# suous/RecNeXt

Hardware: AMD Instinct MI355X
Metric: images/sec RecNeXt-M3 224x224 bf16 (higher is better)
Workload: dtype bf16

## Files before the change

### recnext_amd/csrc/rcx_api.hip

```cpp
#include "../../include/recnext_amd.h"
#include "rcx_opts.h"
#include "rcx_launch.h"

#include <cstdarg>
#include <initializer_list>
#include <cstdio>
#include <cstdlib>

namespace {

thread_local char g_err[512] = "";

int fail(int code, const char* fmt, ...)
{
    va_list ap;
    va_start(ap, fmt);
    vsnprintf(g_err, sizeof(g_err), fmt, ap);
    va_end(ap);
    return code;
}

int hip_fail(hipError_t e, const char* what, const char* prefix = "")
{
    snprintf(g_err, sizeof(g_err), "%s%s: %s", prefix, what, hipGetErrorString(e));
// ... 548 lines not shown
}

size_t rcx_recconv2d_train_saved_bytes(int N, int C, int H, int W, int level, int k)
{
    if (!bwd_extents_ok(N, C, H, W, level, k)) return 0;
    return make_train_ladder(N, C, H, W, level, k).saved_total;
}

size_t rcx_recconv2d_bwd_workspace_bytes(int N, int C, int H, int W, int level, int k)
{
    if (!bwd_extents_ok(N, C, H, W, level, k)) return 0;
    return make_train_ladder(N, C, H, W, level, k).bwd_total;
}

int rcx_recconv2d_fwd_train(const void* x, void* y, const float* wpack, const float* bpack, void* saved, size_t saved_bytes,
                            int N, int C, int H, int W, int level, int k, int mode, int dtype, void* stream)
{
    if (int rc = check_common(x, y, N, C, H, W, k, dtype)) return rc;
    if (!wpack) return fail(RCX_ERR_BAD_ARG, "null weight pack");
    if (level < 0 || level > RCX_MAX_LEVEL) return fail(RCX_ERR_BAD_ARG, "level %d outside [0,%d]", level, RCX_MAX_LEVEL);
    if (mode != RCX_MODE_BILINEAR && mode != RCX_MODE_NEAREST) return fail(RCX_ERR_BAD_ARG, "unknown mode %d", mode);
    const TrainLadder L = make_train_ladder(N, C, H, W, level, k);
    if (L.saved_total > 0 && (!saved || saved_bytes < L.saved_total))
        return fail(RCX_ERR_WORKSPACE, "saved-activation buffer too small: need %zu bytes, got %zu", L.saved_total, saved_bytes);
    hipStream_t s = (hipStream_t)stream;
    const int md = mode == RCX_MODE_NEAREST ? 1 : 0;
    const TrainFwdSchedule sch = train_fwd_schedule(N, C, H, W, level, k, mode, dtype);
    if (sch == TRAIN_STEPS) return recconv2d_steps(x, y, wpack, bpack, (char*)saved, L.f_off, L.c_off, L.h, L.w, N, C, level, k, mode, dtype, s, "train fwd: ");
    const hipError_t e = sch == TRAIN_TILED ? rcx::cpt_recconv(x, y, wpack, bpack, N, C, H, level, md, dtype, s, (float*)saved, L.f_off, L.c_off)
                       : sch == TRAIN_CPL14 ? rcx::cpl14_recconv(x, y, wpack, bpack, N, C, md, dtype, s, (float*)saved, L.f_off, L.c_off)
                                            : rcx::cpl7b_recconv(x, y, wpack, bpack, N, C, md, dtype, s, (float*)saved, L.f_off, L.c_off);
    static const char* const what[] = {"train fwd: fused tiled block", "train fwd: fused 14x14 block", "train fwd: fused 7x7 block"};
    return e == hipSuccess ? 0 : hip_fail(e, what[sch]);
}

int rcx_recconv2d_bwd_gy_dtype(int N, int C, int H, int W, int level, int k, int dtype)
{
    if (!bwd_extents_ok(N, C, H, W, level, k) || !known_dtype(dtype)) return RCX_DTYPE_F32;
    if (dtype != RCX_DTYPE_BF16 || C % 4) return RCX_DTYPE_F32;
    return bwd_schedule(make_train_ladder(N, C, H, W, level, k), N, C, level, k, dtype, true).kind != BWD_STEPS ? dtype : RCX_DTYPE_F32;
}

const char* rcx_recconv2d_bwd_plan(int N, int C, int H, int W, int level, int k, int dtype)
{
    static thread_local char desc[64];
    return bwd_plan(desc, N, C, H, W, level, k, dtype, true, "k_recconv_bwd_");
}

int rcx_recconv2d_bwd(const void* x, const void* gy, int gy_dtype, const float* wpack, const float* wpack_flipped, const void* saved,
                      void* gx, float* gwpack, float* gbpack, void* const* gw_out, void* const* gb_out, int grad_dtype,
                      void* workspace, size_t workspace_bytes,
                      int N, int C, int H, int W, int level, int k, int mode, int dtype, void* stream)
{
    if (int rc = check_common(x, gx, N, C, H, W, k, dtype)) return rc;
    if (!gy || !wpack || !wpack_flipped || (!gwpack && !gw_out)) return fail(RCX_ERR_BAD_ARG, "null gradient / weight pointer");
    if (gw_out && !known_dtype(grad_dtype)) return fail(RCX_ERR_BAD_ARG, "unknown gradient dtype %d", grad_dtype);
    if (int rc = check_bwd_args(gy_dtype, C, level, mode)) return rc;
    const TrainLadder L = make_train_ladder(N, C, H, W, level, k);
    if (level >= 1 && !saved) return fail(RCX_ERR_BAD_ARG, "null saved-activation buffer");
    if (!workspace || workspace_bytes < L.bwd_total)
        return fail(RCX_ERR_WORKSPACE, "backward workspace too small: need %zu bytes, got %zu", L.bwd_total, workspace_bytes);
    const BwdSchedule sch = bwd_schedule(L, N, C, level, k, dtype, true);
    if (gy_dtype != RCX_DTYPE_F32 && !(sch.kind != BWD_STEPS && gy_dtype == dtype && dtype == RCX_DTYPE_BF16))
        return fail(RCX_ERR_UNSUPPORTED, "gy of dtype %d: this problem takes float32 (rcx_recconv2d_bwd_gy_dtype)", gy_dtype);
    if (gw_out)
        for (int i = 0; i < level + 2; ++i)
            if (!gw_out[i]) return fail(RCX_ERR_BAD_ARG, "null gw_out[%d]", i);
    hipStream_t s = (hipStream_t)stream;
    BwdRun B{L, true, "bwd: "};
    B.x = x; B.gy = gy; B.wpack = wpack; B.wflip = wpack_flipped; B.saved = (const char*)saved; B.ws = (char*)workspace; B.gx = gx;
    B.gy_dt = gy_dtype; B.N = N; B.C = C; B.level = level; B.k = k; B.mode = mode; B.dtype = dtype; B.s = s;
    rcx::WgradJobs& J = B.J;
    J.njobs = level + 2; J.kk = k * k; J.C = C; J.param_layout = gw_out ? 1 : 0; J.param_dt = grad_dtype;
    for (int i = 0; i < level + 2; ++i) {
        J.gw[i] = gw_out ? (float*)gw_out[i] : gwpack + (size_t)i * k * k * C;
        J.gb[i] = gw_out ? (gb_out ? (float*)gb_out[i] : nullptr) : (gbpack ? gbpack + (size_t)i * C : nullptr);
    }
    if (sch.kind == BWD_ONE) RCX_TRY(one_launch(B, gy, gy_dtype, gx, 0, H, level, dtype), "fused block", B.prefix);
    else if (int rc = sch.kind == BWD_TILED ? bwd_tiled(B, sch.m) : bwd_steps(B, sch.m)) return rc;
    float* const gw0 = J.gw[0], * const gb0 = J.gb[0];
    if (level == 0) { J.njobs = 1; J.gw[0] = J.gw[1]; J.gb[0] = J.gb[1]; J.nslots[0] = J.nslots[1]; J.part[0][0] = J.part[1][0]; J.rows[0][0] = J.rows[1][0]; }
    RCX_TRY(rcx::bwd_wgrad_reduce_jobs(J, s), "weight-gradient reduction", B.prefix);
    if (level >= 1) return 0;
    const size_t esz = gw_out && grad_dtype != RCX_DTYPE_F32 ? 2 : 4;
    hipError_t e = hipMemsetAsync(gw0, 0, esz * k * k * C, s);
    if (e == hipSuccess && gb0) e = hipMemsetAsync(gb0, 0, esz * C, s);
    return e == hipSuccess ? 0 : hip_fail(e, "bwd: zero down grad");
}

size_t rcx_recconv2d_bwd_input_workspace_bytes(int N, int C, int H, int W, int level, int k)
{
    if (!bwd_extents_ok(N, C, H, W, level, k)) return 0;
    const TrainLadder L = make_train_ladder(N, C, H, W, level, k);
    return bwd_input_workspace(L, bwd_schedule(L, N, C, level, k, RCX_DTYPE_F32, false).kind);
}

int rcx_recconv2d_bwd_input_gy_dtype(int N, int C, int H, int W, int level, int k, int dtype)
{
    if (!bwd_extents_ok(N, C, H, W, level, k) || !known_dtype(dtype) || dtype == RCX_DTYPE_F32 || C % 4) return RCX_DTYPE_F32;
    return bwd_schedule(make_train_ladder(N, C, H, W, level, k), N, C, level, k, dtype, false).kind != BWD_STEPS ? dtype : RCX_DTYPE_F32;
}

const char* rcx_recconv2d_bwd_input_plan(int N, int C, int H, int W, int level, int k, int dtype)
{
    static thread_local char desc[64];
    return bwd_plan(desc, N, C, H, W, level, k, dtype, false, "k_recconv_adj_");
}

int rcx_recconv2d_bwd_input(const void* gy, int gy_dtype, const float* wpack, const float* wpack_flipped, void* gx,
                            void* workspace, size_t workspace_bytes,
                            int N, int C, int H, int W, int level, int k, int mode, int dtype, void* stream)
{
    if (int rc = check_common(gy, gx, N, C, H, W, k, dtype)) return rc;
    if (!wpack || !wpack_flipped) return fail(RCX_ERR_BAD_ARG, "null weight pack");
    if (gy == gx) return fail(RCX_ERR_BAD_ARG, "gx must not alias gy");
    if (int rc = check_bwd_args(gy_dtype, C, level, mode)) return rc;
    const TrainLadder L = make_train_ladder(N, C, H, W, level, k);
    const BwdSchedule sch = bwd_schedule(L, N, C, level, k, dtype, false);
    const size_t need = bwd_input_workspace(L, sch.kind);
    if (need && (!workspace || workspace_bytes < need))
        return fail(RCX_ERR_WORKSPACE, "input-backward workspace too small: need %zu bytes, got %zu", need, workspace_bytes);
    if (gy_dtype != RCX_DTYPE_F32 && !(sch.kind != BWD_STEPS && gy_dtype == dtype))
        return fail(RCX_ERR_UNSUPPORTED, "gy of dtype %d: this problem takes float32 (rcx_recconv2d_bwd_input_gy_dtype)", gy_dtype);
    BwdRun B{L, false, "bwd input: "};
    B.gy = gy; B.gx = gx; B.wpack = wpack; B.wflip = wpack_flipped; B.ws = (char*)workspace;
    B.gy_dt = gy_dtype; B.N = N; B.C = C; B.level = level; B.k = k; B.mode = mode; B.dtype = dtype; B.s = (hipStream_t)stream;
    if (sch.kind == BWD_ONE) RCX_TRY(one_launch(B, gy, gy_dtype, gx, 0, H, level, dtype), "fused block", B.prefix);
    else return sch.kind == BWD_TILED ? bwd_tiled(B, sch.m) : bwd_steps(B, sch.m);
    return 0;
}

#undef RCX_TRY

int rcx_dwconv2d_fwd(const void* x, void* y, const float* w_kkc, const float* bias,
                     int N, int C, int H, int W, int k, int stride, int in_dtype, int out_dtype, void* stream)
{
    if (int rc = check_common(x, y, N, C, H, W, k, in_dtype)) return rc;
    if (!known_dtype(out_dtype)) return fail(RCX_ERR_BAD_ARG, "unknown dtype %d", out_dtype);
    if (!w_kkc) return fail(RCX_ERR_BAD_ARG, "null weight");
    if (stride != 1 && stride != 2) return fail(RCX_ERR_UNSUPPORTED, "stride %d not supported (1 or 2)", stride);
    hipError_t e = step_dwconv(x, y, w_kkc, bias, N, C, H, W, k, stride, in_dtype, out_dtype, (hipStream_t)stream);
    return e == hipSuccess ? 0 : hip_fail(e, "rcx_dwconv2d_fwd");
}

int rcx_dwconv2d_mult2_fwd(const void* x, void* y, const float* w_kkc, const float* bias,
                           int N, int Cin, int H, int W, int k, int stride, int dtype, void* stream)
{
    if (int rc = check_common(x, y, N, Cin, H, W, k, dtype)) return rc;
    if (!w_kkc) return fail(RCX_ERR_BAD_ARG, "null weight");
    if (stride != 1 && stride != 2) return fail(RCX_ERR_UNSUPPORTED, "stride %d not supported (1 or 2)", stride);
    hipError_t e;
    const bool lanes_ok = !rcx::opt::hand_kernels_off() && rcx::down_lanes_applicable(N, Cin, H, W, k, stride, dtype);
    const bool tiled_ok = !rcx::opt::hand_kernels_off() && rcx::down7m2_cpt_applicable(N, Cin, H, W, k, stride, dtype);
    if (tiled_ok && (!lanes_ok || H > 64 || W > 64 || (H <= 14 && W <= 14) || upcpt_everywhere()))
        e = rcx::down7m2_cpt(x, y, w_kkc, bias, N, Cin, H, W, dtype, (hipStream_t)stream);
    else if (lanes_ok)
        e = rcx::down_lanes(x, y, w_kkc, bias, N, Cin, H, W, k, stride, dtype, (hipStream_t)stream);
    else
        e = rcx::generic_dwconv_mult2(x, y, w_kkc, bias, N, Cin, H, W, k, stride, dtype, (hipStream_t)stream);
    return e == hipSuccess ? 0 : hip_fail(e, "rcx_dwconv2d_mult2_fwd");
}

const char* rcx_upadd_dwconv_fwd_plan(int N, int C, int H, int W, int Hc, int Wc, int k, int mode, int x_dtype, int coarse_dtype, int out_dtype, int has_coarse)
{
    if (N <= 0 || C <= 0 || H <= 0 || W <= 0 || k <= 0 || (k & 1) == 0) return "invalid";
    static thread_local char desc[160];
    switch (pick_upadd(N, C, H, W, Hc, Wc, k, x_dtype, coarse_dtype, out_dtype, has_coarse != 0)) {
    case STEP_CPL14: return H == 7 ? "upadd_cpl14(k_upadd_cpl7)" : "upadd_cpl14(k_upadd_cpl14)";
    case STEP_CPT: return rcx::upadd_cpt_describe(N, C, H, W, mode == RCX_MODE_NEAREST ? 1 : 0, x_dtype, desc, (int)sizeof(desc)) > 0 ? desc : "upadd_cpt(k_upadd_cpt)";
    case STEP_LANES: return "upadd_lanes(k_upadd_lanes)";
    case STEP_CONV5_LANES: return "conv5_lanes(k_upadd_lanes)";
    default: return "generic";
    }
}

int rcx_upadd_dwconv_fwd(const void* x, const void* coarse, void* y, const float* w_kkc, const float* bias,
                         int N, int C, int H, int W, int Hc, int Wc, int k, int mode,
                         int x_dtype, int coarse_dtype, int out_dtype, void* stream)
{
    if (int rc = check_common(x, y, N, C, H, W, k, x_dtype)) return rc;
    if (!known_dtype(out_dtype)) return fail(RCX_ERR_BAD_ARG, "unknown dtype %d", out_dtype);
    if (!w_kkc) return fail(RCX_ERR_BAD_ARG, "null weight");
    if (mode != RCX_MODE_BILINEAR && mode != RCX_MODE_NEAREST) return fail(RCX_ERR_BAD_ARG, "unknown mode %d", mode);
    if (coarse) {
        if (Hc <= 0 || Wc <= 0) return fail(RCX_ERR_BAD_ARG, "non-positive coarse extent %dx%d", Hc, Wc);
        if (!known_dtype(coarse_dtype)) return fail(RCX_ERR_BAD_ARG, "unknown dtype %d", coarse_dtype);
    }
    hipError_t e = step_upadd(x, coarse, y, w_kkc, bias, N, C, H, W, Hc, Wc, k, mode, x_dtype, coarse_dtype, out_dtype, (hipStream_t)stream);
    return e == hipSuccess ? 0 : hip_fail(e, "rcx_upadd_dwconv_fwd");
}

namespace {

int check_dw_bwd(const char* who, bool have_ptrs, int N, int C, int H, int W, int dtype, int c_mult)
{
    if (!have_ptrs) return fail(RCX_ERR_BAD_ARG, "%s: null pointer", who);
    if (N <= 0 || C <= 0 || H <= 0 || W <= 0) return fail(RCX_ERR_BAD_ARG, "non-positive extent N=%d C=%d H=%d W=%d", N, C, H, W);
    if (!known_dtype(dtype)) return fail(RCX_ERR_BAD_ARG, "unknown dtype %d", dtype);
    if (C % c_mult) return fail(RCX_ERR_UNSUPPORTED, "%s: the backward kernels need C %% %d == 0, got C=%d", who, c_mult, C);
    return 0;
}

hipError_t reduce_one(const float* part, int rows, float* gw, float* gb, int k, int C, hipStream_t s)
{
    rcx::WgradJobs J{};
    J.njobs = 1; J.kk = k * k; J.C = C;
    J.nslots[0] = 1; J.part[0][0] = part; J.rows[0][0] = rows; J.gw[0] = gw; J.gb[0] = gb;
    return rcx::bwd_wgrad_reduce_jobs(J, s);
}

bool dw_bwd_tiled_gx(int N, int C, int H, int W, int k, int stride)
{
    return stride == 2 && !rcx::opt::hand_kernels_off() && rcx::bwd_cpt_applicable(N, C, H, W, k) && down_size(H, k) * 2 == H && down_size(W, k) * 2 == W;
}

bool dw_bwd_tiled_gw(int N, int C, int H, int W, int k, int stride) { return dw_bwd_tiled_gx(N, C, H, W, k, stride) && N * (H / 14) <= 512; }

bool upadd_bwd_tiled(int N, int C, int H, int W, int Hc, int Wc, int k)
{
    return !rcx::opt::hand_kernels_off() && rcx::bwd_cpt_applicable(N, C, H, W, k) && Hc * 2 == H && Wc * 2 == W;
}

}

size_t rcx_dwconv2d_bwd_workspace_bytes(int C, int k)
{
    if (C <= 0 || k <= 0 || (k & 1) == 0) return 0;
    return align256(rcx::wgrad_partial_bytes(C, k));
}

int rcx_dwconv2d_bwd(const void* x, const float* gy, const float* w_kkc, const float* w_flipped_kkc,
                     void* gx, float* gw, float* gb, void* workspace, size_t workspace_bytes,
                     int N, int C, int H, int W, int k, int stride, int x_dtype, void* stream)
{
    if (k <= 0 || (k & 1) == 0) return fail(RCX_ERR_BAD_ARG, "kernel_size must be odd and positive, got %d", k);
    if (int rc = check_dw_bwd("rcx_dwconv2d_bwd", x && gy && gw, N, C, H, W, x_dtype, 4)) return rc;
    if (stride != 1 && stride != 2) return fail(RCX_ERR_UNSUPPORTED, "stride %d not supported (1 or 2)", stride);
    if (gx && (!w_kkc || !w_flipped_kkc)) return fail(RCX_ERR_BAD_ARG, "rcx_dwconv2d_bwd: weights are needed for the input gradient");
    const size_t need = rcx_dwconv2d_bwd_workspace_bytes(C, k);
    if (!workspace || workspace_bytes < need) return fail(RCX_ERR_WORKSPACE, "workspace too small: need %zu bytes, got %zu", need, workspace_bytes);
    hipStream_t s = (hipStream_t)stream;
    const int p = k / 2, Ho = (H + 2 * p - k) / stride + 1, Wo = (W + 2 * p - k) / stride + 1;
    hipError_t e;
    if (gx) {
        if (stride == 1) e = step_dwconv(gy, gx, w_flipped_kkc, nullptr, N, C, H, W, k, 1, RCX_DTYPE_F32, x_dtype, s);
        else if (dw_bwd_tiled_gx(N, C, H, W, k, stride)) e = rcx::bwd_dT_cpt(gy, gx, x_dtype, w_kkc, N, C, H, s);
        else e = rcx::bwd_down_input(nullptr, gy, gx, x_dtype, w_kkc, N, C, H, W, Ho, Wo, k, s);
        if (e != hipSuccess) return hip_fail(e, "rcx_dwconv2d_bwd: input gradient");
    }
    int rows = 0;
    if (!dw_bwd_tiled_gw(N, C, H, W, k, stride))
        e = rcx::bwd_wgrad(x, x_dtype, nullptr, gy, (float*)workspace, gw, gb, N, C, H, W, 0, 0, Ho, Wo, k, stride, 0, 0, s);
    else if ((e = rcx::bwd_wgrad_d_cpt(x, x_dtype, gy, (float*)workspace, N, C, H, s, &rows)) == hipSuccess)
        e = reduce_one((const float*)workspace, rows, gw, gb, k, C, s);
    return e == hipSuccess ? 0 : hip_fail(e, "rcx_dwconv2d_bwd: weight gradient");
}

size_t rcx_upadd_dwconv_bwd_workspace_bytes(int N, int C, int H, int W, int Hc, int Wc, int k)
{
    if (N <= 0 || C <= 0 || H <= 0 || W <= 0 || k <= 0 || (k & 1) == 0) return 0;
    if (upadd_bwd_tiled(N, C, H, W, Hc, Wc, k)) return align256(sizeof(float) * (size_t)N * ((H + 13) / 14) * (size_t)(k * k + 1) * C);
    return align256(rcx::wgrad_partial_bytes(C, k)) + align256(sizeof(float) * (size_t)N * C * H * W);
}

int rcx_upadd_dwconv_bwd_gy_dtype(int N, int C, int H, int W, int Hc, int Wc, int k, int dtype)
{
    if (dtype != RCX_DTYPE_BF16 || N <= 0 || C <= 0 || C % 4 || k <= 0 || (k & 1) == 0) return RCX_DTYPE_F32;
    return upadd_bwd_tiled(N, C, H, W, Hc, Wc, k) ? dtype : RCX_DTYPE_F32;
}

int rcx_upadd_dwconv_bwd(const void* x, const float* coarse, const void* gy, int gy_dtype, const float* w_kkc, const float* w_flipped_kkc,
                         void* gx, float* gcoarse, float* gw, float* gb, void* workspace, size_t workspace_bytes,
                         int N, int C, int H, int W, int Hc, int Wc, int k, int mode, int dtype, void* stream)
{
    if (Hc <= 0 || Wc <= 0) return fail(RCX_ERR_BAD_ARG, "non-positive coarse extent %dx%d", Hc, Wc);
    if (k <= 0 || (k & 1) == 0) return fail(RCX_ERR_BAD_ARG, "kernel_size must be odd and positive, got %d", k);
    if (!known_dtype(gy_dtype)) return fail(RCX_ERR_BAD_ARG, "unknown dtype %d", gy_dtype);
    if (mode != RCX_MODE_BILINEAR && mode != RCX_MODE_NEAREST) return fail(RCX_ERR_BAD_ARG, "unknown mode %d", mode);
    if (int rc = check_dw_bwd("rcx_upadd_dwconv_bwd", x && coarse && gy && gw && w_flipped_kkc, N, C, H, W, dtype, 4)) return rc;
    const size_t need = rcx_upadd_dwconv_bwd_workspace_bytes(N, C, H, W, Hc, Wc, k);
    if (!workspace || workspace_bytes < need) return fail(RCX_ERR_WORKSPACE, "workspace too small: need %zu bytes, got %zu", need, workspace_bytes);
    const bool tiled = upadd_bwd_tiled(N, C, H, W, Hc, Wc, k);
    if (gy_dtype != RCX_DTYPE_F32 && !(tiled && gy_dtype == dtype && dtype == RCX_DTYPE_BF16))
        return fail(RCX_ERR_UNSUPPORTED, "gy of dtype %d: this problem takes float32 (rcx_upadd_dwconv_bwd_gy_dtype)", gy_dtype);
    hipStream_t s = (hipStream_t)stream;
    float* part = (float*)workspace;
    hipError_t e;
    if (tiled) {
        const int md = mode == RCX_MODE_NEAREST ? 1 : 0;
        if (gcoarse) {
            e = rcx::bwd_gc_cpt(gy, gy_dtype, gcoarse, w_flipped_kkc, N, C, H, md, s);
            if (e != hipSuccess) return hip_fail(e, "rcx_upadd_dwconv_bwd: coarse gradient");
        }
        if (gx) {
            e = rcx::bwd_gx_cpt(gy, gy_dtype, nullptr, gx, dtype, w_flipped_kkc, nullptr, N, C, H, s);
            if (e != hipSuccess) return hip_fail(e, "rcx_upadd_dwconv_bwd: input gradient");
        }
        int rows = 0;
        e = rcx::bwd_wgrad_k_cpt(x, dtype, coarse, gy, gy_dtype, part, N, C, H, md, s, &rows);
        if (e == hipSuccess) e = reduce_one(part, rows, gw, gb, k, C, s);
        return e == hipSuccess ? 0 : hip_fail(e, "rcx_upadd_dwconv_bwd: weight gradient");
    }
    const float* gyf = (const float*)gy;
    float* gT = (float*)((char*)workspace + align256(rcx::wgrad_partial_bytes(C, k)));
    if (gcoarse) {
        e = step_dwconv(gyf, gT, w_flipped_kkc, nullptr, N, C, H, W, k, 1, RCX_DTYPE_F32, RCX_DTYPE_F32, s);
        if (e == hipSuccess) e = rcx::bwd_resize(gT, gcoarse, N, C, H, W, Hc, Wc, mode, s);
// ... 440 lines not shown
```

### recnext_amd/csrc/rcx_upcpt.hip

```cpp
#include "rcx_cpt_kernel.h"
#include "rcx_opts.h"

namespace rcx {
namespace upcpt {

using namespace cpt;

static inline int tile_width(int W, int x_dt) { return (W % 14 != 0 && W % 16 == 0 && x_dt == 1) ? 16 : 14; }

constexpr int NR = 18;

template <int MODE, int TW, int AHEAD> struct Sched {
    static constexpr int NCOL = TW + 4, NCR = TW / 2 + 4, NSTORE = TW;
    static constexpr int c_last = MODE == 0 ? 8 : 7;
    static constexpr bool is_build(int ri) { return MODE == 0 ? (ri & 1) == 1 : ((ri & 1) == 0 && ri >= 2); }
    static constexpr int build_row(int ri) { return MODE == 0 ? (ri - 1) / 2 : (ri - 2) / 2; }
    static constexpr int pending(int kind, int ri_target)
    {
        int seq = 0, xend[NR + AHEAD + 1] = {}, cend[16] = {};
        for (int i = -2; i <= 0; ++i) { seq += NCR; cend[i + 2] = seq; }
        for (int r = 0; r < AHEAD; ++r) { seq += NCOL; xend[r] = seq; }
        if (kind == 0) return seq - cend[1];
        for (int ri = 0; ri < NR; ++ri) {
            if (ri + AHEAD < NR) { seq += NCOL; xend[ri + AHEAD] = seq; }
// ... 372 lines not shown
    const int lane = (int)(threadIdx.x & 63);
    const unsigned upp = (unsigned)(TR * TCn);
    const unsigned wg = (upp & 3u) == 0 ? xcd_workgroup(blockIdx.x, upp >> 2, total / upp) : blockIdx.x;
    const unsigned unit = __builtin_amdgcn_readfirstlane(wg * 4 + (threadIdx.x >> 6));
    if (unit >= total) return;
    const int tc = (int)(unit % (unsigned)TCn);
    unsigned q = unit / (unsigned)TCn;
    const int tr = (int)(q % (unsigned)TR);
    q /= (unsigned)TR;
    const int cb = (int)(q % (unsigned)nb), n = (int)(q / (unsigned)nb);
    const int c = cb * 64 + lane;
    const bool cvalid = c < C;
    const int cc = cvalid ? c : C - 1;
    const unsigned OOB = 0x80000000u;
    const unsigned long long xbase = (unsigned long long)(reinterpret_cast<const char*>(x) + (size_t)n * H * W * pix);
    const unsigned long long ybase = (unsigned long long)(reinterpret_cast<char*>(y) + (size_t)n * Ho * Wo * pixo);
    const unsigned voffM = (unsigned)((TW * tc) * pix + cc * ESZ);
    const unsigned voffL = voffM - 2u * (unsigned)pix;
    const unsigned voffR = voffM + (unsigned)TW * (unsigned)pix;
    auto load_row = [&](uint32_t (&raw)[NCOL], int r) {
        int ar = 14 * tr + r;
        ar = ar < 0 ? 0 : (ar > H - 1 ? H - 1 : ar);
        xrow_load<TIO, PIXB>(raw, voffL, voffM, voffR, row_desc(xbase, ar, H, W * pix), 0, pix);
    };
    auto row_valid = [&](int r) -> bool { const int ar = 14 * tr + r; return ar >= 0 && ar < H; };
    uint32_t raw[NR1][NCOL];
    sfor<AHEAD>([&](auto rc) { load_row(raw[decltype(rc)::value], -2 + decltype(rc)::value); });
    const __amdgpu_buffer_rsrc_t wsrc = __builtin_amdgcn_make_buffer_rsrc((void*)w, 0, 25 * C * 4, 0x00020000);
    Taps td;
    load_taps(td, wsrc, __builtin_amdgcn_make_buffer_rsrc((void*)bias, 0, has_bias ? C * 4 : 0, 0x00020000), 0, C, cc);
#pragma unroll
    for (int u = 0; u < 5; ++u) { pin(td.p[u][0]); pin(td.p[u][1]); pin(td.p[u][2]); }
    f32x2 b0 = f32x2{td.bias, 0.f};
    pin(b0);
    const unsigned yoff = cvalid ? (unsigned)((NPO * tc) * pixo + c * OSZ) : OOB;
    f32x2 facc[3][NPO];
    sfor<NR1>([&](auto rc) {
        constexpr int ri = decltype(rc)::value, r = ri - 2;
        if constexpr (ri + AHEAD < NR1) load_row(raw[ri + AHEAD], r + AHEAD);
        xrow_pin<S::cap(S::pending(ri))>(raw[ri]);
        f32x2 xr[NHP];
#pragma unroll
        for (int k = 0; k < NHP; ++k) xr[k] = f32x2{raw_f32<TIO>(raw[ri][2 * k]), raw_f32<TIO>(raw[ri][2 * k + 1])};
        const bool rv = row_valid(r);
#pragma unroll
        for (int o = 0; o < 7; ++o) {
            const int u = r - 2 * o + 2;
            if (u < 0 || u > 4) continue;
            f32x2(&a)[NPO] = facc[o % 3];
            if (rv) {
#pragma unroll
                for (int i = 0; i < NPO; ++i) a[i] = pfma(xr[i], td.p[u][0], u == 0 ? b0 : a[i]);
#pragma unroll
                for (int i = 0; i < NPO; ++i) a[i] = pfma(xr[i + 1], td.p[u][1], a[i]);
#pragma unroll
                for (int i = 0; i < NPO; ++i) a[i].x = fmaf(xr[i + 2].x, td.p[u][2].x, a[i].x);
            } else if (u == 0) {
#pragma unroll
                for (int i = 0; i < NPO; ++i) a[i] = b0;
            }
            if (u == 4) {
                float out[NPO];
#pragma unroll
                for (int i = 0; i < NPO; ++i) out[i] = a[i].x + a[i].y;
                DownSt<TO>::st(out, yoff, row_desc(ybase, 7 * tr + o, Ho, Wo * pixo), 0, pixo);
            }
        }
#pragma unroll
        for (int o = 0; o < 7; ++o) if (r - 2 * o + 2 >= 0 && r - 2 * o + 2 < 4) pin(facc[o % 3]);
        CPT_FENCE;
    });
}

template <typename TIO, typename TO>
static hipError_t launch_down(const void* x, void* y, const float* w, const float* b, int N, int C, int H, int W, hipStream_t s)
{
    const int tw = tile_width(W, std::is_same<TIO, bf16_t>::value ? 1 : 0);
    const long long units = (long long)N * ((C + 63) / 64) * ((H + 13) / 14) * ((W + tw - 1) / tw);
    const dim3 grid((unsigned)((units + 3) / 4)), block(256);
    const int hb = b != nullptr;
    const int pixb = C * (int)sizeof(TIO);
#define RCX_GO(PB, TW) hipLaunchKernelGGL((k_down5_cpt<PB, TIO, TO, TW>), grid, block, 0, s, (const TIO*)x, (TO*)y, w, b, N, C, H, W, hb)
    if constexpr (std::is_same<TIO, bf16_t>::value) {
        if (tw == 16) {
            if (pixb == 128) RCX_GO(128, 16);
            else if (pixb == 256) RCX_GO(256, 16);
            else RCX_GO(0, 16);
            return hipGetLastError();
        }
    }
    if constexpr (sizeof(TIO) == 2) {
        if (pixb == 128) { RCX_GO(128, 14); return hipGetLastError(); }
        if (pixb == 256) { RCX_GO(256, 14); return hipGetLastError(); }
    }
    RCX_GO(0, 14);
#undef RCX_GO
    return hipGetLastError();
}

#define DN7_ROW_IMM(OP)                                                                                                              \
    "s_add_i32 %[t], %[rb], 0\n\t"                                                                                                  \
    CPT_LI(OP, 0, "vl", "t", 0) CPT_LI(OP, 1, "vl", "t", 1) CPT_LI(OP, 2, "vl", "t", 2)                                              \
    CPT_LI(OP, 3, "vm", "t", 0) CPT_LI(OP, 4, "vm", "t", 1) CPT_LI(OP, 5, "vm", "t", 2) CPT_LI(OP, 6, "vm", "t", 3)                  \
    CPT_LI(OP, 7, "vm", "t", 4) CPT_LI(OP, 8, "vm", "t", 5) CPT_LI(OP, 9, "vm", "t", 6) CPT_LI(OP, 10, "vm", "t", 7)                 \
    CPT_LI(OP, 11, "vm", "t", 8) CPT_LI(OP, 12, "vm", "t", 9) CPT_LI(OP, 13, "vm", "t", 10) CPT_LI(OP, 14, "vm", "t", 11)            \
    CPT_LI(OP, 15, "vm", "t", 12) CPT_LI(OP, 16, "vm", "t", 13)                                                                      \
    CPT_LI(OP, 17, "vr", "t", 0) CPT_LI(OP, 18, "vr", "t", 1) CPT_LI(OP, 19, "vr", "t", 2)
#define DN7_N(OP, d, V) "s_add_i32 %[t2], %[t2], %[pix]\n\t" CPT_LG(OP, d, V, "t2")
#define DN7_ROW_GEN(OP)                                                                                                              \
    "s_add_i32 %[t2], %[rb], 0\n\t" CPT_LG(OP, 0, "vl", "t2") DN7_N(OP, 1, "vl") DN7_N(OP, 2, "vl")                                    \
    "s_add_i32 %[t2], %[rb], 0\n\t" CPT_LG(OP, 17, "vr", "t2") DN7_N(OP, 18, "vr") DN7_N(OP, 19, "vr")                                 \
    "s_add_i32 %[t2], %[rb], 0\n\t" CPT_LG(OP, 3, "vm", "t2") DN7_N(OP, 4, "vm") DN7_N(OP, 5, "vm") DN7_N(OP, 6, "vm") DN7_N(OP, 7, "vm")   \
    DN7_N(OP, 8, "vm") DN7_N(OP, 9, "vm") DN7_N(OP, 10, "vm") DN7_N(OP, 11, "vm") DN7_N(OP, 12, "vm") DN7_N(OP, 13, "vm") DN7_N(OP, 14, "vm") \
    DN7_N(OP, 15, "vm") DN7_N(OP, 16, "vm")
template <typename TIO, int PIXB>
__device__ __forceinline__ void row_load7(uint32_t (&v)[20], unsigned vl, unsigned vm, unsigned vr, i32x4 rs, int rb, int pix)
{
    int t, t2;
    if constexpr (PIXB > 0 && PIXB * 13 <= 4095) {
        (void)pix; (void)t2;
        if constexpr (std::is_same<TIO, f16_t>::value)
            asm volatile(DN7_ROW_IMM(CPT_LDH) : CPT_OUT20(v), [t] "=&s"(t) : [vl] "v"(vl), [vm] "v"(vm), [vr] "v"(vr), [rs] "s"(rs), [rb] "s"(rb), [pb] "n"(PIXB) : "scc");
        else if constexpr (sizeof(TIO) == 2)
            asm volatile(DN7_ROW_IMM(CPT_LD16) : CPT_OUT20(v), [t] "=&s"(t) : [vl] "v"(vl), [vm] "v"(vm), [vr] "v"(vr), [rs] "s"(rs), [rb] "s"(rb), [pb] "n"(PIXB) : "scc");
        else
            asm volatile(DN7_ROW_IMM(CPT_LD32) : CPT_OUT20(v), [t] "=&s"(t) : [vl] "v"(vl), [vm] "v"(vm), [vr] "v"(vr), [rs] "s"(rs), [rb] "s"(rb), [pb] "n"(PIXB) : "scc");
    } else {
        (void)t;
        if constexpr (std::is_same<TIO, f16_t>::value)
            asm volatile(DN7_ROW_GEN(CPT_LDH) : CPT_OUT20(v), [t2] "=&s"(t2) : [vl] "v"(vl), [vm] "v"(vm), [vr] "v"(vr), [rs] "s"(rs), [rb] "s"(rb), [pix] "s"(pix) : "scc");
        else if constexpr (sizeof(TIO) == 2)
            asm volatile(DN7_ROW_GEN(CPT_LD16) : CPT_OUT20(v), [t2] "=&s"(t2) : [vl] "v"(vl), [vm] "v"(vm), [vr] "v"(vr), [rs] "s"(rs), [rb] "s"(rb), [pix] "s"(pix) : "scc");
        else
            asm volatile(DN7_ROW_GEN(CPT_LD32) : CPT_OUT20(v), [t2] "=&s"(t2) : [vl] "v"(vl), [vm] "v"(vm), [vr] "v"(vr), [rs] "s"(rs), [rb] "s"(rb), [pix] "s"(pix) : "scc");
    }
}

constexpr int NR7 = 19;
template <int AHEAD> struct SchedDown7 {
    static constexpr int pending(int ri_target)
    {
        int seq = 0, xend[NR7 + AHEAD + 1] = {};
        for (int r = 0; r < AHEAD; ++r) { seq += 20; xend[r] = seq; }
        for (int ri = 0; ri < NR7; ++ri) {
            if (ri + AHEAD < NR7) { seq += 20; xend[ri + AHEAD] = seq; }
            if (ri == ri_target) return seq - xend[ri];
            if (ri >= 6 && (ri & 1) == 0) seq += 7;
        }
        return 0;
    }
    static constexpr int cap(int v) { return v > 63 ? 63 : v; }
};

template <int PIXB, typename TIO>
__global__ __launch_bounds__(256, 2) void k_down7m2_cpt(const TIO* __restrict__ x, TIO* __restrict__ y, const float* __restrict__ w, const float* __restrict__ bias,
                                                        int N, int Cin, int H, int W, int has_bias)
{
    constexpr int ESZ = (int)sizeof(TIO), AHEAD = 2;
    using S = SchedDown7<AHEAD>;
    const int Co = 2 * Cin, nb = (Co + 63) / 64, TR = (H + 13) / 14, TCn = (W + 13) / 14, Ho = H / 2, Wo = W / 2;
    const int pix = PIXB ? PIXB : Cin * ESZ, pixo = Co * ESZ;
    const unsigned total = (unsigned)N * nb * TR * TCn;
    const int lane = (int)(threadIdx.x & 63);
    const unsigned upp = (unsigned)(TR * TCn);
    const unsigned wg = (upp & 3u) == 0 ? xcd_workgroup(blockIdx.x, upp >> 2, total / upp) : blockIdx.x;
    const unsigned unit = __builtin_amdgcn_readfirstlane(wg * 4 + (threadIdx.x >> 6));
    if (unit >= total) return;
    const int tc = (int)(unit % (unsigned)TCn);
    unsigned q = unit / (unsigned)TCn;
    const int tr = (int)(q % (unsigned)TR);
    q /= (unsigned)TR;
    const int ob = (int)(q % (unsigned)nb), n = (int)(q / (unsigned)nb);
    const int o = ob * 64 + lane;
    const bool ovalid = o < Co;
    const int oo = ovalid ? o : Co - 1;
    const unsigned OOB = 0x80000000u;
    const unsigned long long xbase = (unsigned long long)(reinterpret_cast<const char*>(x) + (size_t)n * H * W * pix);
    const unsigned long long ybase = (unsigned long long)(reinterpret_cast<char*>(y) + (size_t)n * Ho * Wo * pixo);
    const unsigned voffM = (unsigned)((14 * tc) * pix + (oo >> 1) * ESZ);
    const unsigned voffL = voffM - 3u * (unsigned)pix;
    const unsigned voffR = voffM + 14u * (unsigned)pix;
    auto load_row = [&](uint32_t (&raw)[20], int r) { row_load7<TIO, PIXB>(raw, voffL, voffM, voffR, row_desc(xbase, 14 * tr + r, H, W * pix), 0, pix); };
    uint32_t raw[NR7][20];
    sfor<AHEAD>([&](auto rc) { load_row(raw[decltype(rc)::value], -3 + decltype(rc)::value); });
    const __amdgpu_buffer_rsrc_t wsrc = __builtin_amdgcn_make_buffer_rsrc((void*)w, 0, 49 * Co * 4, 0x00020000);
    f32x2 tp[7][4];
#pragma unroll
    for (int u = 0; u < 7; ++u) {
#pragma unroll
        for (int v = 0; v < 7; ++v) {
            const float wv = __uint_as_float(__builtin_amdgcn_raw_buffer_load_b32(wsrc, oo * 4, (u * 7 + v) * Co * 4, 0));
            if (v & 1) tp[u][v >> 1].y = wv;
            else tp[u][v >> 1].x = wv;
        }
        tp[u][3].y = 0.f;
    }
#pragma unroll
    for (int u = 0; u < 7; ++u) { pin(tp[u][0]); pin(tp[u][1]); pin(tp[u][2]); pin(tp[u][3]); }
    f32x2 b0 = f32x2{has_bias ? bias[oo] : 0.f, 0.f};
    pin(b0);
    const unsigned yoff = ovalid ? (unsigned)((7 * tc) * pixo + o * ESZ) : OOB;
    f32x2 facc[4][7];
    sfor<NR7>([&](auto rc) {
        constexpr int ri = decltype(rc)::value, r = ri - 3;
        if constexpr (ri + AHEAD < NR7) load_row(raw[ri + AHEAD], r + AHEAD);
        pin_row20<S::cap(S::pending(ri))>(raw[ri]);
        f32x2 xr[10];
#pragma unroll
        for (int k = 0; k < 10; ++k) xr[k] = f32x2{raw_f32<TIO>(raw[ri][2 * k]), raw_f32<TIO>(raw[ri][2 * k + 1])};
#pragma unroll
        for (int ot = 0; ot < 7; ++ot) {
            const int u = r - 2 * ot + 3;
            if (u < 0 || u > 6) continue;
            f32x2(&a)[7] = facc[ot % 4];
#pragma unroll
            for (int i = 0; i < 7; ++i) a[i] = pfma(xr[i], tp[u][0], u == 0 ? b0 : a[i]);
#pragma unroll
            for (int i = 0; i < 7; ++i) a[i] = pfma(xr[i + 1], tp[u][1], a[i]);
#pragma unroll
            for (int i = 0; i < 7; ++i) a[i] = pfma(xr[i + 2], tp[u][2], a[i]);
#pragma unroll
            for (int i = 0; i < 7; ++i) a[i].x = fmaf(xr[i + 3].x, tp[u][3].x, a[i].x);
            if (u == 6) {
                float out[7];
#pragma unroll
                for (int i = 0; i < 7; ++i) out[i] = a[i].x + a[i].y;
                DownSt<TIO>::st(out, yoff, row_desc(ybase, 7 * tr + ot, Ho, Wo * pixo), 0, pixo);
            }
        }
#pragma unroll
        for (int ot = 0; ot < 7; ++ot) if (r - 2 * ot + 3 >= 0 && r - 2 * ot + 3 < 6) pin(facc[ot % 4]);
        CPT_FENCE;
    });
}

template <typename TIO>
static hipError_t launch_down7(const void* x, void* y, const float* w, const float* b, int N, int Cin, int H, int W, hipStream_t s)
{
    const long long units = (long long)N * ((2 * Cin + 63) / 64) * ((H + 13) / 14) * ((W + 13) / 14);
    const dim3 grid((unsigned)((units + 3) / 4)), block(256);
    const int hb = b != nullptr;
    const int pixb = Cin * (int)sizeof(TIO);
#define RCX_GO(PB) hipLaunchKernelGGL((k_down7m2_cpt<PB, TIO>), grid, block, 0, s, (const TIO*)x, (TIO*)y, w, b, N, Cin, H, W, hb)
    if constexpr (sizeof(TIO) == 2) {
        if (pixb == 128) { RCX_GO(128); return hipGetLastError(); }
        if (pixb == 256) { RCX_GO(256); return hipGetLastError(); }
    }
    RCX_GO(0);
#undef RCX_GO
    return hipGetLastError();
}

static inline bool enabled() { return !rcx::opt::off(rcx::opt::UPADD_CPT) && !rcx::opt::hand_kernels_off(); }

template <int MODE, typename TIO, typename TC>
static hipError_t launch(const void* x, const void* coarse, void* y, const float* w, const float* b, int N, int C, int H, int W, hipStream_t s)
{
    const int tw = tile_width(W, std::is_same<TIO, bf16_t>::value ? 1 : 0);
    const long long units = (long long)N * ((C + 63) / 64) * ((H + 13) / 14) * ((W + tw - 1) / tw);
    const dim3 grid((unsigned)((units + 3) / 4)), block(256);
    const int hb = b != nullptr;
    const int pixb = C * (int)sizeof(TIO);
#define RCX_GO(PB, TW) hipLaunchKernelGGL((k_upadd_cpt<MODE, PB, TIO, TC, TW>), grid, block, 0, s, (const TIO*)x, (const TC*)coarse, (TIO*)y, w, b, N, C, H, W, hb)
    if constexpr (std::is_same<TIO, bf16_t>::value) {
        if (tw == 16) {
            if (pixb == 128) RCX_GO(128, 16);
            else if (pixb == 256) RCX_GO(256, 16);
            else RCX_GO(0, 16);
            return hipGetLastError();
        }
    }
    if constexpr (sizeof(TIO) == 2) {
        if (pixb == 128) { RCX_GO(128, 14); return hipGetLastError(); }
        if (pixb == 256) { RCX_GO(256, 14); return hipGetLastError(); }
    }
    RCX_GO(0, 14);
#undef RCX_GO
    return hipGetLastError();
}

}

bool upadd_cpt_applicable(int N, int C, int H, int W, int Hc, int Wc, int k, int x_dt, int c_dt, int out_dt)
{
    if (!upcpt::enabled() || k != 5 || out_dt != x_dt || x_dt < 0 || x_dt > 2 || !(c_dt == x_dt || c_dt == 0)) return false;
    const int tw = upcpt::tile_width(W, x_dt);
    if (N < 1 || C < 1 || Hc * 2 != H || Wc * 2 != W || H < 28 || W < 28) return false;
    const long long img = (long long)H * W * C * 4;
    const long long units = (long long)N * ((C + 63) / 64) * ((H + 13) / 14) * ((W + tw - 1) / tw);
    return img < (1ll << 31) && units < (1ll << 31);
}

int upadd_cpt_describe(int N, int C, int H, int W, int mode, int x_dt, char* buf, int len)
{
    const int pixb = x_dt != 0 && (C == 64 || C == 128) ? C * 2 : 0, tw = upcpt::tile_width(W, x_dt);
    return snprintf(buf, len, "upadd_cpt(k_upadd_cpt<%d, %d>,tw=%d,cb=64,nt=256,tiles=%lld)", mode, pixb, tw,
                    (long long)N * ((C + 63) / 64) * ((H + 13) / 14) * ((W + tw - 1) / tw));
}

hipError_t upadd_cpt(const void* x, const void* coarse, void* y, const float* w, const float* b, int N, int C, int H, int W, int mode,
                     int x_dt, int c_dt, hipStream_t s)
{
#define RCX_UP(TX, TC) (mode == 1 ? upcpt::launch<1, TX, TC>(x, coarse, y, w, b, N, C, H, W, s) : upcpt::launch<0, TX, TC>(x, coarse, y, w, b, N, C, H, W, s))
    if (x_dt == 1) return c_dt == 1 ? RCX_UP(bf16_t, bf16_t) : RCX_UP(bf16_t, float);
    if (x_dt == 2) return c_dt == 2 ? RCX_UP(f16_t, f16_t) : RCX_UP(f16_t, float);
    return RCX_UP(float, float);
#undef RCX_UP
}

bool down5_cpt_applicable(int N, int C, int H, int W, int k, int stride, int in_dt, int out_dt)
{
    if (!upcpt::enabled() || k != 5 || stride != 2 || in_dt < 0 || in_dt > 2 || !(out_dt == in_dt || out_dt == 0)) return false;
    const int tw = upcpt::tile_width(W, in_dt);
    if (N < 1 || C < 1 || (H & 1) || (W & 1) || H < 28 || W < 28) return false;
    const long long img = (long long)H * W * C * 4;
    const long long units = (long long)N * ((C + 63) / 64) * ((H + 13) / 14) * ((W + tw - 1) / tw);
    return img < (1ll << 31) && units < (1ll << 31);
}

hipError_t down5_cpt(const void* x, void* y, const float* w, const float* b, int N, int C, int H, int W, int in_dt, int out_dt, hipStream_t s)
{
    if (in_dt == 1) return out_dt == 1 ? upcpt::launch_down<bf16_t, bf16_t>(x, y, w, b, N, C, H, W, s) : upcpt::launch_down<bf16_t, float>(x, y, w, b, N, C, H, W, s);
    if (in_dt == 2) return out_dt == 2 ? upcpt::launch_down<f16_t, f16_t>(x, y, w, b, N, C, H, W, s) : upcpt::launch_down<f16_t, float>(x, y, w, b, N, C, H, W, s);
    return upcpt::launch_down<float, float>(x, y, w, b, N, C, H, W, s);
}

bool down7m2_cpt_applicable(int N, int Cin, int H, int W, int k, int stride, int dtype)
{
    if (!upcpt::enabled() || k != 7 || stride != 2 || dtype < 0 || dtype > 2) return false;
    if (N < 1 || Cin < 1 || (H & 1) || (W & 1) || H < 14 || W < 14) return false;
    const long long img = (long long)H * W * Cin * 4;
    const long long units = (long long)N * ((2 * Cin + 63) / 64) * ((H + 13) / 14) * ((W + 13) / 14);
    return img < (1ll << 31) && units < (1ll << 31);
}

hipError_t down7m2_cpt(const void* x, void* y, const float* w, const float* b, int N, int Cin, int H, int W, int dtype, hipStream_t s)
{
    if (dtype == 1) return upcpt::launch_down7<bf16_t>(x, y, w, b, N, Cin, H, W, s);
    if (dtype == 2) return upcpt::launch_down7<f16_t>(x, y, w, b, N, Cin, H, W, s);
    return upcpt::launch_down7<float>(x, y, w, b, N, Cin, H, W, s);
}

}
```

Baseline: 129,900.

## Compute both channel-multiplier outputs per lane in stride-2 7x7 down conv

The stride-2 depthwise 7x7 channel-multiplier-2 kernel now maps each lane to one input channel and computes both of its output channels as a packed f32x2, instead of one output channel per lane. This halves input loads and the number of work units, and uses op_sel packed FMAs to pick even or odd input columns. Stores are packed pairs written by new inline-asm store helpers. The dispatcher is also changed so that the tiled kernel is used everywhere except 32x32 inputs, where the lanes kernel is kept. The cost is more weight registers per lane (7x7 pairs instead of 7x4), which may reduce occupancy.

```diff
diff --git a/recnext_amd/csrc/rcx_api.hip b/recnext_amd/csrc/rcx_api.hip
--- a/recnext_amd/csrc/rcx_api.hip
+++ b/recnext_amd/csrc/rcx_api.hip
@@ -724,7 +724,8 @@
     hipError_t e;
     const bool lanes_ok = !rcx::opt::hand_kernels_off() && rcx::down_lanes_applicable(N, Cin, H, W, k, stride, dtype);
     const bool tiled_ok = !rcx::opt::hand_kernels_off() && rcx::down7m2_cpt_applicable(N, Cin, H, W, k, stride, dtype);
-    if (tiled_ok && (!lanes_ok || H > 64 || W > 64 || (H <= 14 && W <= 14) || upcpt_everywhere()))
+    const bool lanes_wins = lanes_ok && H == 32 && W == 32;
+    if (tiled_ok && (!lanes_wins || upcpt_everywhere()))
         e = rcx::down7m2_cpt(x, y, w_kkc, bias, N, Cin, H, W, dtype, (hipStream_t)stream);
     else if (lanes_ok)
         e = rcx::down_lanes(x, y, w_kkc, bias, N, Cin, H, W, k, stride, dtype, (hipStream_t)stream);
diff --git a/recnext_amd/csrc/rcx_upcpt.hip b/recnext_amd/csrc/rcx_upcpt.hip
--- a/recnext_amd/csrc/rcx_upcpt.hip
+++ b/recnext_amd/csrc/rcx_upcpt.hip
@@ -548,13 +548,47 @@
     static constexpr int cap(int v) { return v > 63 ? 63 : v; }
 };
 
+template <int HI> __device__ __forceinline__ f32x2 bfma(f32x2 xp, f32x2 t, f32x2 c)
+{
+    f32x2 d;
+    if constexpr (HI) asm("v_pk_fma_f32 %0, %1, %2, %3 op_sel:[1,0,0] op_sel_hi:[1,1,1]" : "=v"(d) : "v"(xp), "v"(t), "v"(c));
+    else asm("v_pk_fma_f32 %0, %1, %2, %3 op_sel:[0,0,0] op_sel_hi:[0,1,1]" : "=v"(d) : "v"(xp), "v"(t), "v"(c));
+    return d;
+}
+
+template <typename TIO> struct PairSt {
+    static __device__ __forceinline__ void st(const f32x2 (&a)[7], unsigned vo, i32x4 rs, int rb, int pix)
+    {
+        int t;
+        if constexpr (sizeof(TIO) == 2) {
+            uint32_t p[7];
+#pragma unroll
+            for (int j = 0; j < 7; ++j) {
+                if constexpr (std::is_same<TIO, f16_t>::value) asm("v_cvt_pk_f16_f32 %0, %1, %2" : "=v"(p[j]) : "v"(a[j].x), "v"(a[j].y));
+                else asm("v_cvt_pk_bf16_f32 %0, %1, %2" : "=v"(p[j]) : "v"(a[j].x), "v"(a[j].y));
+            }
+            asm volatile("s_add_i32 %[t], %[rb], 0\n\t" DN_S("buffer_store_dword", 0) DN_N DN_S("buffer_store_dword", 1) DN_N DN_S("buffer_store_dword", 2) DN_N
+                         DN_S("buffer_store_dword", 3) DN_N DN_S("buffer_store_dword", 4) DN_N DN_S("buffer_store_dword", 5) DN_N DN_S("buffer_store_dword", 6)
+                         : [t] "=&s"(t)
+                         : [p0] "v"(p[0]), [p1] "v"(p[1]), [p2] "v"(p[2]), [p3] "v"(p[3]), [p4] "v"(p[4]), [p5] "v"(p[5]), [p6] "v"(p[6]),
+                           [vo] "v"(vo), [rs] "s"(rs), [rb] "s"(rb), [pix] "s"(pix) : "scc", "memory");
+        } else {
+            asm volatile("s_add_i32 %[t], %[rb], 0\n\t" DN_S("buffer_store_dwordx2", 0) DN_N DN_S("buffer_store_dwordx2", 1) DN_N DN_S("buffer_store_dwordx2", 2) DN_N
+                         DN_S("buffer_store_dwordx2", 3) DN_N DN_S("buffer_store_dwordx2", 4) DN_N DN_S("buffer_store_dwordx2", 5) DN_N DN_S("buffer_store_dwordx2", 6)
+                         : [t] "=&s"(t)
+                         : [p0] "v"(a[0]), [p1] "v"(a[1]), [p2] "v"(a[2]), [p3] "v"(a[3]), [p4] "v"(a[4]), [p5] "v"(a[5]), [p6] "v"(a[6]),
+                           [vo] "v"(vo), [rs] "s"(rs), [rb] "s"(rb), [pix] "s"(pix) : "scc", "memory");
+        }
+    }
+};
+
 template <int PIXB, typename TIO>
 __global__ __launch_bounds__(256, 2) void k_down7m2_cpt(const TIO* __restrict__ x, TIO* __restrict__ y, const float* __restrict__ w, const float* __restrict__ bias,
                                                         int N, int Cin, int H, int W, int has_bias)
 {
     constexpr int ESZ = (int)sizeof(TIO), AHEAD = 2;
     using S = SchedDown7<AHEAD>;
-    const int Co = 2 * Cin, nb = (Co + 63) / 64, TR = (H + 13) / 14, TCn = (W + 13) / 14, Ho = H / 2, Wo = W / 2;
+    const int Co = 2 * Cin, nb = (Cin + 63) / 64, TR = (H + 13) / 14, TCn = (W + 13) / 14, Ho = H / 2, Wo = W / 2;
     const int pix = PIXB ? PIXB : Cin * ESZ, pixo = Co * ESZ;
     const unsigned total = (unsigned)N * nb * TR * TCn;
     const int lane = (int)(threadIdx.x & 63);
@@ -566,36 +600,31 @@
     unsigned q = unit / (unsigned)TCn;
     const int tr = (int)(q % (unsigned)TR);
     q /= (unsigned)TR;
-    const int ob = (int)(q % (unsigned)nb), n = (int)(q / (unsigned)nb);
-    const int o = ob * 64 + lane;
-    const bool ovalid = o < Co;
-    const int oo = ovalid ? o : Co - 1;
+    const int cb = (int)(q % (unsigned)nb), n = (int)(q / (unsigned)nb);
+    const int c = cb * 64 + lane;
+    const bool cvalid = c < Cin;
+    const int cc = cvalid ? c : Cin - 1;
     const unsigned OOB = 0x80000000u;
     const unsigned long long xbase = (unsigned long long)(reinterpret_cast<const char*>(x) + (size_t)n * H * W * pix);
     const unsigned long long ybase = (unsigned long long)(reinterpret_cast<char*>(y) + (size_t)n * Ho * Wo * pixo);
-    const unsigned voffM = (unsigned)((14 * tc) * pix + (oo >> 1) * ESZ);
+    const unsigned voffM = (unsigned)((14 * tc) * pix + cc * ESZ);
     const unsigned voffL = voffM - 3u * (unsigned)pix;
     const unsigned voffR = voffM + 14u * (unsigned)pix;
     auto load_row = [&](uint32_t (&raw)[20], int r) { row_load7<TIO, PIXB>(raw, voffL, voffM, voffR, row_desc(xbase, 14 * tr + r, H, W * pix), 0, pix); };
     uint32_t raw[NR7][20];
     sfor<AHEAD>([&](auto rc) { load_row(raw[decltype(rc)::value], -3 + decltype(rc)::value); });
     const __amdgpu_buffer_rsrc_t wsrc = __builtin_amdgcn_make_buffer_rsrc((void*)w, 0, 49 * Co * 4, 0x00020000);
-    f32x2 tp[7][4];
+    f32x2 tp[7][7];
 #pragma unroll
     for (int u = 0; u < 7; ++u) {
 #pragma unroll
-        for (int v = 0; v < 7; ++v) {
-            const float wv = __uint_as_float(__builtin_amdgcn_raw_buffer_load_b32(wsrc, oo * 4, (u * 7 + v) * Co * 4, 0));
-            if (v & 1) tp[u][v >> 1].y = wv;
-            else tp[u][v >> 1].x = wv;
-        }
-        tp[u][3].y = 0.f;
-    }
-#pragma unroll
-    for (int u = 0; u < 7; ++u) { pin(tp[u][0]); pin(tp[u][1]); pin(tp[u][2]); pin(tp[u][3]); }
-    f32x2 b0 = f32x2{has_bias ? bias[oo] : 0.f, 0.f};
+        for (int v = 0; v < 7; ++v) tp[u][v] = __builtin_bit_cast(f32x2, __builtin_amdgcn_raw_buffer_load_b64(wsrc, cc * 8, (u * 7 + v) * Co * 4, 0));
+    }
+#pragma unroll
+    for (int u = 0; u < 7; ++u) pin(tp[u]);
+    f32x2 b0 = f32x2{has_bias ? bias[2 * cc] : 0.f, has_bias ? bias[2 * cc + 1] : 0.f};
     pin(b0);
-    const unsigned yoff = ovalid ? (unsigned)((7 * tc) * pixo + o * ESZ) : OOB;
+    const unsigned yoff = cvalid ? (unsigned)((7 * tc) * pixo + 2 * c * ESZ) : OOB;
     f32x2 facc[4][7];
     sfor<NR7>([&](auto rc) {
         constexpr int ri = decltype(rc)::value, r = ri - 3;
@@ -609,20 +638,14 @@
             const int u = r - 2 * ot + 3;
             if (u < 0 || u > 6) continue;
             f32x2(&a)[7] = facc[ot % 4];
-#pragma unroll
-            for (int i = 0; i < 7; ++i) a[i] = pfma(xr[i], tp[u][0], u == 0 ? b0 : a[i]);
-#pragma unroll
-            for (int i = 0; i < 7; ++i) a[i] = pfma(xr[i + 1], tp[u][1], a[i]);
-#pragma unroll
-            for (int i = 0; i < 7; ++i) a[i] = pfma(xr[i + 2], tp[u][2], a[i]);
-#pragma unroll
-            for (int i = 0; i < 7; ++i) a[i].x = fmaf(xr[i + 3].x, tp[u][3].x, a[i].x);
-            if (u == 6) {
-                float out[7];
-#pragma unroll
-                for (int i = 0; i < 7; ++i) out[i] = a[i].x + a[i].y;
-                DownSt<TIO>::st(out, yoff, row_desc(ybase, 7 * tr + ot, Ho, Wo * pixo), 0, pixo);
-            }
+            sfor<7>([&](auto vc) {
+                constexpr int v = decltype(vc)::value;
+                sfor<7>([&](auto ic) {
+                    constexpr int i = decltype(ic)::value, j = 2 * i + v;
+                    a[i] = bfma<j & 1>(xr[j >> 1], tp[u][v], (u == 0 && v == 0) ? b0 : a[i]);
+                });
+            });
+            if (u == 6) PairSt<TIO>::st(a, yoff, row_desc(ybase, 7 * tr + ot, Ho, Wo * pixo), 0, pixo);
         }
 #pragma unroll
         for (int ot = 0; ot < 7; ++ot) if (r - 2 * ot + 3 >= 0 && r - 2 * ot + 3 < 6) pin(facc[ot % 4]);
@@ -633,7 +656,7 @@
 template <typename TIO>
 static hipError_t launch_down7(const void* x, void* y, const float* w, const float* b, int N, int Cin, int H, int W, hipStream_t s)
 {
-    const long long units = (long long)N * ((2 * Cin + 63) / 64) * ((H + 13) / 14) * ((W + 13) / 14);
+    const long long units = (long long)N * ((Cin + 63) / 64) * ((H + 13) / 14) * ((W + 13) / 14);
     const dim3 grid((unsigned)((units + 3) / 4)), block(256);
     const int hb = b != nullptr;
     const int pixb = Cin * (int)sizeof(TIO);
@@ -726,7 +749,7 @@
     if (!upcpt::enabled() || k != 7 || stride != 2 || dtype < 0 || dtype > 2) return false;
     if (N < 1 || Cin < 1 || (H & 1) || (W & 1) || H < 14 || W < 14) return false;
     const long long img = (long long)H * W * Cin * 4;
-    const long long units = (long long)N * ((2 * Cin + 63) / 64) * ((H + 13) / 14) * ((W + 13) / 14);
+    const long long units = (long long)N * ((Cin + 63) / 64) * ((H + 13) / 14) * ((W + 13) / 14);
     return img < (1ll << 31) && units < (1ll << 31);
 }
 
```

After: 130,600 (median of 6 runs). No clear change (+0.5%).
